# ppwwyyxx/OpenPano

Hardware: AMD Instinct MI355X
Metric: SIFT keypoints+desc/sec and all-pairs matches/sec at 1/2/4/8 GPUs (higher is better)
Workload: dtype f32; 1 GPU; BASELINE config 4 restated: 38 unordered 1300x867 views per GPU (x1 GPUs = a 38-image job); seeded synthetic views (ope~; images_per_gpu=38, images_in_job=38

## Files before the change

openpano_amd/csrc/descriptor.hip:

```cpp
#include "internal.hpp"
#include "devmath.hpp"
#include <stddef.h>

namespace {

typedef float f32x4 __attribute__((ext_vector_type(4)));
#ifndef DESC_WAVES
#define DESC_WAVES 6
#endif
#ifndef DESC_GRID_MULT
#define DESC_GRID_MULT 8
#endif
constexpr int QCAP = 128;
constexpr int COLCAP = 1024;
constexpr int LIST_CAP = OP_DESC_LIST_CAP;
constexpr int ZERO4 = LIST_CAP;

struct DescLds {
	float sorted[LIST_CAP + 4] __attribute__((aligned(16)));
	unsigned long long mask[128];
	float hist[128];
	unsigned short off[128];
	unsigned q[QCAP];
	uint64_t exptab[32];
	unsigned long long startbits[COLCAP / 64];
	unsigned colpk[64];
};
#define WAVE_FENCE() asm volatile("" ::: "memory")

__device__ __forceinline__ int wave_scan_add(int v) {
	v += __builtin_amdgcn_update_dpp(0, v, 0x111, 0xF, 0xF, false);
	v += __builtin_amdgcn_update_dpp(0, v, 0x112, 0xF, 0xF, false);
	v += __builtin_amdgcn_update_dpp(0, v, 0x114, 0xF, 0xF, false);
	v += __builtin_amdgcn_update_dpp(0, v, 0x118, 0xF, 0xF, false);
	v += __builtin_amdgcn_update_dpp(0, v, 0x142, 0xA, 0xF, false);
	v += __builtin_amdgcn_update_dpp(0, v, 0x143, 0xC, 0xF, false);
	return v;
}
__device__ __forceinline__ int wave_max_i(int v) {
	int t;
	t = __builtin_amdgcn_update_dpp(0, v, 0x111, 0xF, 0xF, false); v = t > v ? t : v;
	t = __builtin_amdgcn_update_dpp(0, v, 0x112, 0xF, 0xF, false); v = t > v ? t : v;
	t = __builtin_amdgcn_update_dpp(0, v, 0x114, 0xF, 0xF, false); v = t > v ? t : v;
	t = __builtin_amdgcn_update_dpp(0, v, 0x118, 0xF, 0xF, false); v = t > v ? t : v;
	t = __builtin_amdgcn_update_dpp(0, v, 0x142, 0xA, 0xF, false); v = t > v ? t : v;
	t = __builtin_amdgcn_update_dpp(0, v, 0x143, 0xC, 0xF, false); v = t > v ? t : v;
	return __builtin_amdgcn_readlane(v, 63);
}

__device__ __forceinline__ int rank_below(unsigned long long m) {
	return (int)__builtin_amdgcn_mbcnt_hi((unsigned)(m >> 32), __builtin_amdgcn_mbcnt_lo((unsigned)m, 0u));
}

__device__ __forceinline__ int uni(int v) { return __builtin_amdgcn_readfirstlane(v); }
__device__ __forceinline__ float uni(float v) { return __builtin_bit_cast(float, __builtin_amdgcn_readfirstlane(__builtin_bit_cast(int, v))); }
__device__ __forceinline__ double uni(double v) {
	const unsigned long long b = __builtin_bit_cast(unsigned long long, v);
	const unsigned lo = (unsigned)__builtin_amdgcn_readfirstlane((int)(unsigned)b), hi = (unsigned)__builtin_amdgcn_readfirstlane((int)(unsigned)(b >> 32));
	return __builtin_bit_cast(double, ((unsigned long long)hi << 32) | lo);
}

__global__ void __launch_bounds__(64) __attribute__((amdgpu_waves_per_eu(DESC_WAVES, DESC_WAVES))) k_descriptor(SiftPlan p, const KeyPoint* __restrict__ oriented,
		const long long* __restrict__ total_ptr, long long cap, float* __restrict__ desc, double* __restrict__ coor, double* __restrict__ real) {
	__shared__ DescLds S;
	const int lane = threadIdx.x;
	const float pi2 = (float)(2 * 3.14159265358979323846);
	const float nbin_per_rad = 8 / pi2;
	S.mask[lane] = 0ULL; S.mask[lane + 64] = 0ULL;
	if (lane < 4) S.sorted[ZERO4 + lane] = 0.f;
	if (lane < 32) S.exptab[lane] = opdev::kExp2fTab[lane];
	const int ownp = (lane & ~7) | ((lane + 7) & 7);
	const int list_cap4 = p.desc_list_cap >> 2;
	__syncthreads();

	long long total = *total_ptr;
	total = total < cap ? total : cap;
	for (long long kk = blockIdx.x; kk < total; kk += gridDim.x) {
		const KeyPoint kp = oriented[kk];
		const int img = uni(kp.pad);
		const int kpx = uni(kp.x), kpy = uni(kp.y), koct = uni(kp.oct), kscale = uni(kp.scale);
		const OctDesc od = p.oct[koct];
		const int w = od.w, h = od.h;
		const float* base = p.ws + (long long)img * p.ws_stride;
		const float* g_img = base + plane_off_gauss(od, p.nscale, kscale);
		const float ort = uni(kp.dir);
		const float hist_w = uni(kp.sf * (float)p.desc_scale_factor);
		const double rd = uni(1.0 / (double)hist_w);
		const float exp_denom = 2 * (4.f * 4.f);
		const int radius = uni((int)round(0.70710678118654752440 * (double)hist_w * (4 + 1)));
		const float cosort = uni(opdev::cosf_glibc(ort)), sinort = uni(opdev::sinf_glibc(ort));
		const int side = 2 * radius + 1, nsamp = side * side;
		const float fr2 = (float)radius * (float)radius;
		S.hist[lane] = 0.f; S.hist[lane + 64] = 0.f;
		int qhead = 0, qn = 0;

		int ncand = nsamp;
		bool cols = side <= 64;
		if (cols) {
			int lo = 0, len = 0;
			if (lane < side) {
				const int xx = lane - radius;
				const float fxx = (float)xx;
				const int nowx = kpx + xx;
				const float yc = floorf(sqrtf(fr2 - fxx * fxx) + 1e-3f);
				float ylo = -yc, yhi = yc;
				const float m = 0.005f * hist_w + 0.05f;
				const float blo = -2.5f * hist_w - m, bhi = 1.5f * hist_w + m;
				if (fabsf(cosort) > 0.01f) {
					const float rc = 1.f / cosort;
					const float a = (blo + fxx * sinort) * rc, b = (bhi + fxx * sinort) * rc;
					ylo = fmaxf(ylo, fminf(a, b)); yhi = fminf(yhi, fmaxf(a, b));
				}
				if (fabsf(sinort) > 0.01f) {
					const float rs = 1.f / sinort;
					const float a = (blo - fxx * cosort) * rs, b = (bhi - fxx * cosort) * rs;
					ylo = fmaxf(ylo, fminf(a, b)); yhi = fminf(yhi, fmaxf(a, b));
				}
				int ilo = (int)ceilf(ylo), ihi = (int)floorf(yhi);
				ilo = ilo < -radius ? -radius : ilo; ihi = ihi > radius ? radius : ihi;
				ilo = ilo < 1 - kpy ? 1 - kpy : ilo; ihi = ihi > h - 2 - kpy ? h - 2 - kpy : ihi;
				if (nowx >= 1 && nowx <= w - 2 && ihi >= ilo) { lo = ilo; len = ihi - ilo + 1; }
			}
			const int incl = wave_scan_add(len);
			ncand = __builtin_amdgcn_readlane(incl, 63);
			cols = ncand <= COLCAP;
			if (cols) {
				const int start = incl - len;
				const unsigned long long nonempty = __ballot(len > 0);
				unsigned long long zero64 = 0ULL;
				asm volatile("" : "+v"(zero64));
				if (lane < COLCAP / 64) S.startbits[lane] = zero64;
				WAVE_FENCE();
				if (len > 0) {
					atomicOr(&S.startbits[start >> 6], 1ULL << (start & 63));
					S.colpk[rank_below(nonempty)] = ((unsigned)start << 16) | (((unsigned)lo & 0xFFu) << 8) | (unsigned)lane;
				}
			} else ncand = nsamp;
			WAVE_FENCE();
		}

		auto rotate = [&](int xx, int yy, float& x_rot, float& y_rot) {
			const float fxx = (float)xx, fyy = (float)yy;
			y_rot = (float)((double)((float)(-xx) * sinort + fyy * cosort) * rd);
			x_rot = (float)((double)(fxx * cosort + fyy * sinort) * rd);
		};

		auto process_batch = [&](bool cand, int xx, int yy) {
			float x_rot, y_rot;
			rotate(xx, yy, x_rot, y_rot);
			const float ybin = (y_rot + 2.f) - 0.5f, xbin = (x_rot + 2.f) - 0.5f;
			const bool ok = cand && !((float)xx * (float)xx + (float)yy * (float)yy > fr2)
				&& ybin >= -1.f && ybin <= 3.f && xbin >= -1.f && xbin <= 3.f;
			int a0 = 0;
			int a1 = 0;
			float vA[4], vB[4];
			bool vy0 = false, vy1 = false, vx0 = false, vx1 = false;
#pragma unroll
			for (int u = 0; u < 4; ++u) { vA[u] = 0.f; vB[u] = 0.f; }
			if (ok) {
				const int gi = (kpy + yy) * w + (kpx + xx);
				const float gdy = g_img[gi + w] - g_img[gi - w];
				const float gdx = g_img[gi + 1] - g_img[gi - 1];
				const float now_mag = opdev::hypotf_glibc(gdx, gdy);
				float now_ort = opdev::fast_atan_plus_pi(gdy, gdx);
				float weight = opdev::expf_glibc(-(x_rot * x_rot + y_rot * y_rot) / exp_denom, S.exptab);
				weight = weight * now_mag;
				now_ort -= ort;
				if (now_ort < 0) now_ort += pi2;
				if (now_ort > pi2) now_ort -= pi2;
				const float hbin = now_ort * nbin_per_rad;
				const float yf = floorf(ybin), xf = floorf(xbin), hf = floorf(hbin);
				const float ybind = ybin - yf, xbind = xbin - xf, hbind = hbin - hf;
				const float omh = 1 - hbind;
				const int yb = (int)yf, xb = (int)xf;
				vy0 = yb >= 0; vy1 = yb <= 2; vx0 = xb >= 0; vx1 = xb <= 2;
				const int hq8 = ((int)hf & 7) * 8;
				a0 = (yb * 4 + xb) * 64 + hq8;
				a1 = (yb * 4 + xb) * 64 + ((hq8 + 8) & 56);
#pragma unroll
				for (int dy = 0; dy < 2; ++dy) {
					const float w_y = weight * (dy ? ybind : 1 - ybind);
#pragma unroll
					for (int dx = 0; dx < 2; ++dx) {
						const float w_x = w_y * (dx ? xbind : 1 - xbind);
						vA[dy * 2 + dx] = w_x * omh; vB[dy * 2 + dx] = w_x * hbind;
					}
				}
			}
			const bool valid[4] = {vy0 && vx0, vy0 && vx1, vy1 && vx0, vy1 && vx1};
			char* const lds = (char*)&S;
			constexpr int MASK0 = (int)offsetof(DescLds, mask), OFF0 = (int)offsetof(DescLds, off);
			constexpr int CELL_OFF[4] = {0, 1, 4, 5};
#pragma unroll
			for (int u = 0; u < 4; ++u)
				if (valid[u]) atomicOr((unsigned long long*)(lds + MASK0 + a0 + CELL_OFF[u] * 64), 1ULL << lane);
			WAVE_FENCE();
			f32x4* const sorted4 = (f32x4*)S.sorted;
			unsigned* const rec = (unsigned*)S.mask;
			const unsigned long long c0 = S.mask[lane] | S.mask[ownp], c1 = S.mask[lane + 64] | S.mask[ownp + 64];
			unsigned long long u0 = c0, u1 = c1;
			int n0 = (__popcll(u0) + 3) >> 2, n1 = (__popcll(u1) + 3) >> 2;
			int incl = wave_scan_add(n0 + n1);
			const int npass = __builtin_amdgcn_readlane(incl, 63) <= list_cap4 ? 1 : 2;
			for (int pass = 0; pass < npass; ++pass) {
				unsigned long long lm = ~0ULL;
				if (npass == 2) {
					lm = pass == 0 ? 0xFFFFFFFFULL : 0xFFFFFFFF00000000ULL;
					u0 = c0 & lm; u1 = c1 & lm;
					n0 = (__popcll(u0) + 3) >> 2; n1 = (__popcll(u1) + 3) >> 2;
					incl = wave_scan_add(n0 + n1);
				}
				const int q0 = incl - (n0 + n1), q1 = q0 + n0;
				S.off[lane] = (unsigned short)(q0 * 16); S.off[lane + 64] = (unsigned short)(q1 * 16);
				sorted4[n0 ? q0 + n0 - 1 : ZERO4 / 4] = f32x4{0.f, 0.f, 0.f, 0.f};
				sorted4[n1 ? q1 + n1 - 1 : ZERO4 / 4] = f32x4{0.f, 0.f, 0.f, 0.f};
				WAVE_FENCE();
				S.mask[lane] = u0; S.mask[lane + 64] = u1;
				WAVE_FENCE();
				if ((lm >> lane) & 1ULL) {
					const int o0 = a0 >> 2, o1 = a1 >> 2;
#pragma unroll
					for (int u = 0; u < 4; ++u)
						if (valid[u]) {
							const unsigned long long ma = *(const unsigned long long*)(lds + MASK0 + a0 + CELL_OFF[u] * 64);
							const unsigned long long mb = *(const unsigned long long*)(lds + MASK0 + a1 + CELL_OFF[u] * 64);
							const int sa = *(const unsigned short*)(lds + OFF0 + o0 + CELL_OFF[u] * 16);
							const int sb = *(const unsigned short*)(lds + OFF0 + o1 + CELL_OFF[u] * 16);
							*(float*)(lds + sa + rank_below(ma) * 4) = vA[u];
							*(float*)(lds + sb + rank_below(mb) * 4) = vB[u];
						}
				}
				WAVE_FENCE();
				{
					const unsigned long long b0 = __ballot(n0 > 0), b1 = __ballot(n1 > 0);
					const int nb0 = __popcll(b0), nrec = nb0 + __popcll(b1);
					if (n0) rec[rank_below(b0)] = (unsigned)lane | ((unsigned)q0 << 8) | ((unsigned)n0 << 16);
					if (n1) rec[nb0 + rank_below(b1)] = (unsigned)(lane + 64) | ((unsigned)q1 << 8) | ((unsigned)n1 << 16);
					WAVE_FENCE();
					for (int r0 = 0; r0 < nrec; r0 += 64) {
						const unsigned my = r0 + lane < nrec ? rec[r0 + lane] : 0u;
						const int bin = (int)(my & 0xFFu), q = (int)((my >> 8) & 0xFFu), nn = (int)(my >> 16);
						float hsum = S.hist[bin];
						for (int e = 0; __ballot(e < nn) != 0ULL; e += 2) {
							const f32x4 a = sorted4[e < nn ? q + e : ZERO4 / 4], c = sorted4[e + 1 < nn ? q + e + 1 : ZERO4 / 4];
							hsum += a.x; hsum += a.y; hsum += a.z; hsum += a.w; hsum += c.x; hsum += c.y; hsum += c.z; hsum += c.w;
						}
						if (nn) S.hist[bin] = hsum;
					}
				}
				WAVE_FENCE();
			}
			S.mask[lane] = 0ULL; S.mask[lane + 64] = 0ULL;
			WAVE_FENCE();
		};

		int qx = lane / side, qy = lane % side;
		int kbase = -1;
		for (int i0 = 0; i0 < ncand || qn > 0; i0 += 64) {
			bool cand = i0 + lane < ncand, run = true;
			int xx = 0, yy = 0;
			if (cols) {
				const unsigned long long sb = S.startbits[i0 >> 6];
				const int ord = kbase + rank_below(sb) + (int)((unsigned)(sb >> lane) & 1u);
				kbase += __popcll(sb);
				if (cand) {
					const unsigned pk = S.colpk[ord];
					xx = (int)(pk & 0xFFu) - radius; yy = (int)(signed char)(pk >> 8) + (i0 + lane - (int)(pk >> 16));
				}
			} else {
				bool ok = false;
				xx = qx - radius; yy = qy - radius;
				qy += 64; while (qy >= side) { qy -= side; ++qx; }
				const int nowx = kpx + xx, nowy = kpy + yy;
				if (cand && nowx >= 1 && nowx <= w - 2 && nowy >= 1 && nowy <= h - 2) {
					const float fxx = (float)xx, fyy = (float)yy;
					if (!(fxx * fxx + fyy * fyy > fr2)) {
						float x_rot, y_rot;
						rotate(xx, yy, x_rot, y_rot);
						const float ybin = (y_rot + 2.f) - 0.5f, xbin = (x_rot + 2.f) - 0.5f;
						ok = (ybin >= -1.f && ybin <= 3.f && xbin >= -1.f && xbin <= 3.f);
					}
				}
				const unsigned long long mask = __ballot(ok);
				if (ok) S.q[(qhead + qn + rank_below(mask)) & (QCAP - 1)] = (unsigned)(xx + 32768) | ((unsigned)(yy + 32768) << 16);
				qn += __popcll(mask);
				run = qn >= 64 || (i0 + 64 >= ncand && qn > 0);
				if (run) {
					WAVE_FENCE();
					const int n = qn < 64 ? qn : 64;
					const unsigned pk = S.q[(qhead + lane) & (QCAP - 1)];
					cand = lane < n;
					xx = (int)(pk & 0xFFFFu) - 32768; yy = (int)(pk >> 16) - 32768;
					qhead = (qhead + n) & (QCAP - 1); qn -= n;
					WAVE_FENCE();
				}
			}
			if (run) process_batch(cand, xx, yy);
		}

		float* hist = S.hist;
		WAVE_FENCE();
		float sum = 0.f;
#pragma unroll 4
		for (int i = 0; i < 32; ++i) { const f32x4 q = ((const f32x4*)hist)[i]; sum += q.x; sum += q.y; sum += q.z; sum += q.w; }
		float* out = desc + kk * 128;
#pragma unroll
		for (int t = 0; t < 2; ++t) {
			const int i = lane + 64 * t;
			const float v = hist[i] / sum;
			out[i] = sqrtf(v) * (float)p.desc_int_factor;
		}
		if (lane == 0) {
			int sw = p.sw, sh = p.sh;
			asm volatile("" : "+s"(sw), "+s"(sh));
			coor[kk * 2] = (kp.rx - 0.5) * (double)sw;
			coor[kk * 2 + 1] = (kp.ry - 0.5) * (double)sh;
			real[kk * 2] = kp.rx; real[kk * 2 + 1] = kp.ry;
		}
		WAVE_FENCE();
	}
}

}

hipError_t launch_descriptor(const SiftPlan& p, const KeyPoint* oriented, const long long* total,
		long long cap, float* desc, double* coor, double* real, hipStream_t st) {
	if (cap <= 0) return hipSuccess;
	const long long most = (long long)(p.num_cu > 0 ? p.num_cu : 256) * 4 * DESC_WAVES * DESC_GRID_MULT;
	const int grid = (int)(cap < most ? cap : most);
	hipLaunchKernelGGL(k_descriptor, dim3(grid), dim3(64), 0, st, p, oriented, total, cap, desc, coor, real);
	return hipGetLastError();
}
```

Baseline: 50.01 million keypoints+descriptors/s.

## Build descriptor bin masks from factored ballots instead of LDS atomicOr

The descriptor kernel used to build each of 128 bin membership masks with up to four LDS 64-bit atomicOr operations per lane. A separate pass then ORed the mask with the neighbouring orientation bin and cleared it afterwards. The new code takes wave ballots for each y-bin, x-bin and orientation value and merges adjacent ones. It writes the 16 resulting factor masks into LDS with writelane and computes each bin mask as the AND of its y, x and orientation factors. This removes the atomics, the clearing stores and a fence, at the cost of about 26 ballots and some scalar work per batch.

Measured after the change: 50.53 million keypoints+descriptors/s (median of 6 runs). 1.01x the previous value.

```diff
diff --git a/openpano_amd/csrc/descriptor.hip b/openpano_amd/csrc/descriptor.hip
--- a/openpano_amd/csrc/descriptor.hip
+++ b/openpano_amd/csrc/descriptor.hip
@@ -18,6 +18,7 @@
 
 struct DescLds {
 	float sorted[LIST_CAP + 4] __attribute__((aligned(16)));
+	unsigned long long fac[16];
 	unsigned long long mask[128];
 	float hist[128];
 	unsigned short off[128];
@@ -66,10 +67,8 @@
 	const int lane = threadIdx.x;
 	const float pi2 = (float)(2 * 3.14159265358979323846);
 	const float nbin_per_rad = 8 / pi2;
-	S.mask[lane] = 0ULL; S.mask[lane + 64] = 0ULL;
 	if (lane < 4) S.sorted[ZERO4 + lane] = 0.f;
 	if (lane < 32) S.exptab[lane] = opdev::kExp2fTab[lane];
-	const int ownp = (lane & ~7) | ((lane + 7) & 7);
 	const int list_cap4 = p.desc_list_cap >> 2;
 	__syncthreads();
 
@@ -155,6 +154,7 @@
 			int a1 = 0;
 			float vA[4], vB[4];
 			bool vy0 = false, vy1 = false, vx0 = false, vx1 = false;
+			int yb = -8, xb = -8, h0 = -8;
 #pragma unroll
 			for (int u = 0; u < 4; ++u) { vA[u] = 0.f; vB[u] = 0.f; }
 			if (ok) {
@@ -172,9 +172,9 @@
 				const float yf = floorf(ybin), xf = floorf(xbin), hf = floorf(hbin);
 				const float ybind = ybin - yf, xbind = xbin - xf, hbind = hbin - hf;
 				const float omh = 1 - hbind;
-				const int yb = (int)yf, xb = (int)xf;
+				yb = (int)yf; xb = (int)xf; h0 = (int)hf & 7;
 				vy0 = yb >= 0; vy1 = yb <= 2; vx0 = xb >= 0; vx1 = xb <= 2;
-				const int hq8 = ((int)hf & 7) * 8;
+				const int hq8 = h0 * 8;
 				a0 = (yb * 4 + xb) * 64 + hq8;
 				a1 = (yb * 4 + xb) * 64 + ((hq8 + 8) & 56);
 #pragma unroll
@@ -191,13 +191,30 @@
 			char* const lds = (char*)&S;
 			constexpr int MASK0 = (int)offsetof(DescLds, mask), OFF0 = (int)offsetof(DescLds, off);
 			constexpr int CELL_OFF[4] = {0, 1, 4, 5};
-#pragma unroll
-			for (int u = 0; u < 4; ++u)
-				if (valid[u]) atomicOr((unsigned long long*)(lds + MASK0 + a0 + CELL_OFF[u] * 64), 1ULL << lane);
-			WAVE_FENCE();
+			unsigned long long by[5], bx[5], bh[8], AY[4], AX[4], AH[8];
+#pragma unroll
+			for (int k = 0; k < 5; ++k) { by[k] = __ballot(yb == k - 1); bx[k] = __ballot(xb == k - 1); }
+#pragma unroll
+			for (int k = 0; k < 8; ++k) bh[k] = __ballot(h0 == k);
+#pragma unroll
+			for (int k = 0; k < 4; ++k) { AY[k] = by[k + 1] | by[k]; AX[k] = bx[k + 1] | bx[k]; }
+#pragma unroll
+			for (int k = 0; k < 8; ++k) AH[k] = bh[k] | bh[(k + 7) & 7];
 			f32x4* const sorted4 = (f32x4*)S.sorted;
 			unsigned* const rec = (unsigned*)S.mask;
-			const unsigned long long c0 = S.mask[lane] | S.mask[ownp], c1 = S.mask[lane + 64] | S.mask[ownp + 64];
+			{
+				int tlo = 0, thi = 0;
+#pragma unroll
+				for (int k = 0; k < 16; ++k) {
+					const unsigned long long v = k < 4 ? AY[k] : k < 8 ? AX[k - 4] : AH[k - 8];
+					asm("v_writelane_b32 %0, %1, %2" : "+v"(tlo) : "s"((unsigned)v), "n"(k));
+					asm("v_writelane_b32 %0, %1, %2" : "+v"(thi) : "s"((unsigned)(v >> 32)), "n"(k));
+				}
+				if (lane < 16) S.fac[lane] = ((unsigned long long)(unsigned)thi << 32) | (unsigned)tlo;
+			}
+			WAVE_FENCE();
+			const unsigned long long axh = S.fac[4 + ((lane >> 3) & 3)] & S.fac[8 + (lane & 7)];
+			const unsigned long long c0 = S.fac[lane >> 5] & axh, c1 = S.fac[(lane >> 5) + 2] & axh;
 			unsigned long long u0 = c0, u1 = c1;
 			int n0 = (__popcll(u0) + 3) >> 2, n1 = (__popcll(u1) + 3) >> 2;
 			int incl = wave_scan_add(n0 + n1);
@@ -250,8 +267,6 @@
 				}
 				WAVE_FENCE();
 			}
-			S.mask[lane] = 0ULL; S.mask[lane + 64] = 0ULL;
-			WAVE_FENCE();
 		};
 
 		int qx = lane / side, qy = lane % side;
```
